# skit-ai/N-Best-ASR-Transformer

Hardware: AMD Instinct MI355X
Metric: utterances/sec fine-tune (bert-base, seq128, n_best=5) (higher is better)
Workload: dtype bf16

## Files before the change

### include/nbest_hip.h

```cpp
#ifndef NBEST_HIP_H
#define NBEST_HIP_H

#include <stddef.h>
#include <stdint.h>

#ifdef __cplusplus
extern "C" {
#endif

#define NBEST_ABI_VERSION 1

enum { NBEST_OK = 0, NBEST_ERR_ARG = -1, NBEST_ERR_SHAPE = -2, NBEST_ERR_DTYPE = -3, NBEST_ERR_ALIGN = -4,
       NBEST_ERR_LAUNCH = -5, NBEST_ERR_WORKSPACE = -6 };
enum { NBEST_F32 = 0, NBEST_BF16 = 1 };

typedef void* nbest_stream_t;

int nbest_version(void);
int nbest_last_error(char* buf, size_t n);

int nbest_embed_ln_fwd(const int64_t* ids, const int64_t* seg, const int64_t* pos, const void* word,
                       const void* type, const void* ptab, const float* gamma, const float* beta, void* out,
                       float* stats, int64_t M, int H, float eps, int dtype, float drop_p, uint64_t seed,
                       uint32_t drop_stream, nbest_stream_t stream);
// ... 61 lines not shown
  int32_t wave_rows, wave_cols;
  int32_t stages;
  int32_t form;
  int32_t reg_epilogue;
  int32_t splits;
  int64_t k_per_split;
  int32_t b_packed;
  int32_t kernel_epilogue;
} nbest_gemm_plan_info;
int nbest_gemm_plan(const nbest_gemm_args* a, nbest_gemm_plan_info* out);

size_t nbest_wgrad_pair_ws_bytes(const nbest_gemm_args* a, const nbest_gemm_args* b);
int nbest_wgrad_pair(const nbest_gemm_args* a, const nbest_gemm_args* b, nbest_stream_t stream);
int nbest_wgrad_group(const nbest_gemm_args* problems, int n, nbest_stream_t stream);
int nbest_wgrad_window(const nbest_gemm_args* problems, const int32_t* tile_first, const int32_t* tile_count, int n, nbest_stream_t stream);

typedef struct nbest_gemm_fp8_args {
  const void* A;
  const void* B;
  void* C;
  const float* bias;
  const void* R;
  void* U;
  void* C8;
  int64_t M, N, K;
  int64_t lda, ldb, ldc, ldr, ldu, ldc8;
  int32_t epilogue;
  float out_scale;
  float drop_p;
  uint32_t drop_stream;
// ... 221 lines not shown
```

### n-best-asr-transformer_amd/csrc/encoder.hip

```cpp
#include <algorithm>
#include <vector>

#include "common.h"

namespace {

static inline size_t al(size_t x) { return (x + 255) & ~(size_t)255; }
static inline size_t take(size_t& o, size_t bytes) { const size_t at = o; o += bytes; return at; }

struct Sizes {
  size_t esz, MH, MF, M3H, MH8, MF8, st, lse;
  int64_t M;
};

static Sizes sizes(const nbest_encoder_desc* d) {
  Sizes z;
  z.esz = d->dtype == NBEST_BF16 ? 2 : 4;
  z.M = (int64_t)d->B * d->S;
  const size_t MHe = (size_t)z.M * d->H, MFe = (size_t)z.M * d->F;
  z.MH = al(MHe * z.esz); z.MF = al(MFe * z.esz); z.M3H = al(3 * MHe * z.esz);
  z.MH8 = al(MHe); z.MF8 = al(MFe);
  z.st = al((size_t)z.M * 2 * sizeof(float));
  z.lse = al((size_t)d->B * d->heads * d->S * sizeof(float));
  return z;
// ... 263 lines not shown
  g.M = M; g.N = N; g.K = K; g.lda = K; g.ldb = K; g.ldc = N;
  return g;
}

static void use_packed(nbest_gemm_args& g, const void* arena, int64_t off) {
  if (!arena || g.dtype != NBEST_BF16 || g.trans_a || g.trans_b) return;
  g.B_packed = (const char*)arena + off * 2;
  g.b_pack_bn = nbest_pack_bn(g.N);
}
static void use_packed(nbest_gemm_fp8_args& g, const void* arena, int64_t off) {
  if (!arena) return;
  g.B_packed = (const uint8_t*)arena + off;
  g.b_pack_bn = nbest_pack_bn_fp8(g.N, g.K);
}

struct GemmPass {
  int dtype; int64_t M; nbest_stream_t stream;
  uint64_t seed;
  Ptrs W; const void* packed; bool b_kn;
  bool fp8; const void *w8, *w8_packed; const float* inv_scale; const uint32_t* amax_prev; uint32_t* amax_new;
  void* colsum_ws; size_t colsum_ws_bytes; int accumulate;
};
struct GemmOp {
  const void* A; const uint8_t* A8; int a_idx;
  int64_t w_off; int mat;
  void* C; int64_t N, K; int epilogue;
  const float* bias;
  const void* R; float drop_p; uint32_t drop_stream;
  void* U; float* colsum;
  uint8_t* C8; int c_idx;
};

static int layer_gemm(const GemmPass& c, const GemmOp& o) {
  if (c.fp8) {
    nbest_gemm_fp8_args g = {};
    g.A = o.A8; g.B = (const uint8_t*)c.w8 + o.w_off; g.C = o.C; g.bias = o.bias; g.R = o.R; g.U = o.U; g.C8 = o.C8;
// ... 7 lines not shown
      g.c8_amax_prev = c.amax_prev + o.c_idx;
      g.c8_amax_new = c.amax_new ? c.amax_new + (int64_t)o.c_idx * NBEST_AMAX_TENSOR_WORDS : nullptr;
    }
    g.colsum_out = o.colsum; g.colsum_accumulate = c.accumulate; g.ws = c.colsum_ws; g.ws_bytes = c.colsum_ws_bytes;
    return nbest_gemm_fp8(&g, c.stream);
  }
  nbest_gemm_args g = gemm_nt(c.dtype, o.A, c.W.W(o.w_off), o.C, c.M, o.N, o.K);
  if (c.b_kn) { g.trans_b = 1; g.ldb = o.N; }
  g.epilogue = o.epilogue; g.bias = o.bias;
  if (o.R) { g.R = o.R; g.ldr = o.N; }
  if (o.epilogue == NBEST_EPI_BIAS_DROP_RES) { g.drop_p = o.drop_p; g.drop_stream = o.drop_stream; g.seed = c.seed; }
  if (o.epilogue == NBEST_EPI_BIAS_GELU || o.epilogue == NBEST_EPI_DGELU) { g.U = o.U; g.ldu = o.N; }
  if (o.epilogue == NBEST_EPI_DGELU) {
    g.colsum_out = o.colsum; g.colsum_accumulate = g.accumulate = c.accumulate; g.ws = c.colsum_ws; g.ws_bytes = c.colsum_ws_bytes;
  }
  use_packed(g, c.packed, o.w_off);
  return nbest_gemm(&g, c.stream);
}

struct LayerBufs {
  void *qkv, *ctx, *r1, *x1, *u, *hact, *r2;
  float *lse, *st1, *st2;
  uint32_t* keep;
  uint8_t *x8, *ctx8, *x18, *h8;
};

static LayerBufs stashed_layer(const nbest_encoder_desc* d, const ActLayout& a, void* act, int l) {
  char* Lb = (char*)act + a.layer0 + (size_t)(l - a.K) * a.layer_stride;
  LayerBufs b = {};
  b.qkv = Lb + a.o_qkv; b.ctx = Lb + a.o_ctx; b.lse = (float*)(Lb + a.o_lse);
// ... 88 lines not shown
  const nbest_layer_offsets& o = d->layers_host[l];
  const Ptrs& P = c.g.W;
  const nbest_stream_t stream = c.g.stream;
  hipStream_t st = (hipStream_t)stream;
  const int H = d->H, F = d->F, dt = d->dtype, t = 4 * l;
  const int64_t B = d->B, SH = (int64_t)d->S * H;
  const uint32_t s0 = d->drop_stream_base + 1 + 4 * l;
  const bool hdrop = d->hidden_drop > 0.f;
  void* tmp = (char*)b.r2 + (size_t)B * H * P.esz;
  const GemmOp wqkv = {xin, nullptr, t + 0, o.wqkv, t + 0, b.qkv, 3 * H, H, NBEST_EPI_BIAS, P.P(o.bqkv)};
  RUN(layer_gemm(c.g, wqkv));
  RUN(nbest_attention_cls_fwd_internal(b.qkv, SH * 3, (const char*)b.qkv + H * P.esz, 3 * H, c.key_mask, b.ctx, H, d->B, d->S, d->heads, 64, dt,
                                       stream, d->attn_drop, d->seed, s0 + 0));
  auto dense_drop_res = [&](const void* A, int64_t w_off, const float* bias, int64_t N, int64_t K, const void* R, int64_t ldr, uint32_t ds,
                            void* out) -> int {
    nbest_gemm_args g = gemm_nt(dt, A, P.W(w_off), hdrop ? tmp : out, B, N, K);
    g.bias = bias;
    if (hdrop) {
      g.epilogue = NBEST_EPI_BIAS;
      RUN(nbest_gemm(&g, stream));
      return nbest_internal_rows_drop_res(tmp, N, R, ldr, out, N, B, (int)N, d->S, dt, d->hidden_drop, d->seed, ds, st);
    }
    g.epilogue = NBEST_EPI_BIAS_DROP_RES; g.R = R; g.ldr = ldr;
    return nbest_gemm(&g, stream);
  };
  RUN(dense_drop_res(b.ctx, o.wo, P.P(o.bo), H, H, xin, SH, s0 + 1, b.r1));
  RUN(nbest_internal_layernorm_fwd8(b.r1, P.P(o.ln1_g), P.P(o.ln1_b), b.x1, nullptr, b.st1, B, H, d->ln_eps, dt, stream, nullptr, nullptr));
  nbest_gemm_args g = gemm_nt(dt, b.x1, P.W(o.w1), b.hact, B, F, H);
  g.epilogue = NBEST_EPI_BIAS_GELU; g.bias = P.P(o.b1); g.U = b.u; g.ldu = F;
  RUN(nbest_gemm(&g, stream));
  RUN(dense_drop_res(b.hact, o.w2, P.P(o.b2), H, F, b.x1, H, s0 + 2, b.r2));
  RUN(nbest_internal_layernorm_fwd8(b.r2, P.P(o.ln2_g), P.P(o.ln2_b), tmp, nullptr, b.st2, B, H, d->ln_eps, dt, stream, nullptr, nullptr));
  return nbest_internal_rows_drop_res(tmp, H, nullptr, 0, xout, SH, B, H, 1, dt, 0.f, 0, 0, st);
}

}

extern "C" size_t nbest_encoder_act_bytes(const nbest_encoder_desc* d) { return d ? act_layout(d, sizes(d)).total : 0; }

extern "C" int nbest_encoder_act_view(const nbest_encoder_desc* d, void* act, int layer, void** qkv, float** lse) {
  RUN(check_desc(d));
  RUN(check_cls_top(d));
  NB_CHECK(act && qkv && lse, NBEST_ERR_ARG, "encoder_act_view: null pointer");
  NB_CHECK(0 <= layer && layer < d->L, NBEST_ERR_ARG, "encoder_act_view: layer %d outside [0, L=%d)", layer, d->L);
  const ActLayout a = act_layout(d, sizes(d));
// ... 203 lines not shown
    void *dR2 = dR, *dR1 = dR, *dRd2 = dRd, *dRd1 = dRd, *dBigL = dBig, *dqkvL = dqkv;
    if (deferred) {
      dRd2 = W + w.gset[gpos][0]; dBigL = W + w.gset[gpos][1]; dRd1 = W + w.gset[gpos][2]; dqkvL = W + w.gset[gpos][3];
      if (!hdrop) { dR2 = dRd2; dR1 = dRd1; }
    }
    const bool cls = cls_layer_of(d, l);
    if (cls) {
      const size_t bh = (size_t)d->B * H * z.esz;
      dR2 = W + w.dR; dR1 = W + w.dB1 + bh; dBigL = dBig;
      dRd2 = hdrop ? (void*)(W + w.dRd) : dR2; dRd1 = hdrop ? (void*)(W + w.dRd + bh) : dR1;
    }
    const WGrad wg[4] = {{dqkvL, X(l), dqkv8, b.x8, o.wqkv, 3 * H, H, t + 3, t + 0},
                         {dRd1, b.ctx, dRd8, b.ctx8, o.wo, H, H, t + 2, t + 1},
                         {dBigL, b.x1, dBig8, b.x18, o.w1, F, H, t + 1, t + 2},
                         {dRd2, b.hact, dRd8, b.h8, o.w2, H, F, t + 0, t + 3}};
    auto cls_wgrad = [&](int j) -> int {
      if (frozen(l, j)) return NBEST_OK;
      nbest_gemm_args g = wgrad_args(dt, wg[j].rows, wg[j].cols, d->B);
      g.A = wg[j].dY; g.B = wg[j].X; g.C = G(wg[j].w_off); g.accumulate = accumulate;
      g.ws = slab; g.ws_bytes = w.slab_bytes;
      return nbest_gemm(&g, stream);
    };
    auto cls_wgrads = [&]() -> int {
      RUN(cls_wgrad(3));
      RUN(cls_wgrad(2));
      return cls_wgrad(1);
    };
    if (!npg) nbest_internal_rowred_batch_begin();
    if (cls) {
      const int64_t Bn = d->B, SH = (int64_t)d->S * H;
      const size_t bh = (size_t)Bn * H * z.esz, half = w.red_bytes / 2;
      void* dAc = W + w.dR + bh;
      GemmPass dgc = dg;
      dgc.M = Bn; dgc.packed = nullptr;
      const Fp8Grad nof8 = {nullptr, nullptr, nullptr};
      RUN(nbest_internal_rows_drop_res(dA, SH, nullptr, 0, dAc, H, Bn, H, 1, dt, 0.f, 0, 0, st));
      RUN(nbest_internal_layernorm_bwd8(dAc, b.r2, b.st2, P.P(o.ln2_g), dR2, nullptr, G(o.ln2_g), G(o.ln2_b), hdrop ? nullptr : G(o.b2), Bn, H, dt,
                                        accumulate, 0.f, 0, 0, red, half, stream, nof8));
      if (hdrop) {
        RUN(nbest_internal_rows_drop_res(dR2, H, nullptr, 0, dRd2, H, Bn, H, d->S, dt, d->hidden_drop, d->seed, s0 + 2, st));
        RUN(nbest_colsum(dRd2, G(o.b2), Bn, H, H, dt, accumulate, (char*)red + half, half, stream));
      }
      GemmOp dw2 = {dRd2, nullptr, t + 0, o.w2, t + 3, dBigL, F, H, NBEST_EPI_DGELU};
      dw2.U = b.u; dw2.colsum = G(o.b1);
      RUN(layer_gemm(dgc, dw2));
      GemmOp dw1 = {dBigL, nullptr, t + 1, o.w1, t + 2, dB1, H, F, NBEST_EPI_RES};
      dw1.R = dR2;
      RUN(layer_gemm(dgc, dw1));
      RUN(nbest_internal_layernorm_bwd8(dB1, b.r1, b.st1, P.P(o.ln1_g), dR1, nullptr, G(o.ln1_g), G(o.ln1_b), hdrop ? nullptr : G(o.bo), Bn, H, dt,
// ... 57 lines not shown
        const WinLaunch& wl = wp.launches[wi];
        nbest_gemm_args tab[kWinEntries];
        int32_t first[kWinEntries], count[kWinEntries];
        for (int i = 0; i < wl.n; ++i) {
          tab[i] = wargs[(size_t)4 * (layer_end - 1 - wl.e[i].layer) + wl.e[i].j];
          first[i] = wl.e[i].first; count[i] = wl.e[i].count;
        }
        pair_begin();
        RUN(nbest_wgrad_window(tab, first, count, wl.n, stream));
        pair_end();
      }
      pair_end();
      if (l == layer_begin)
        for (; pairs_used < nl; ++pairs_used) { stamp(0); stamp(1); }
    } else if (!grouped && cls) {
      stamp(0); RUN(cls_wgrad(3)); stamp(1);
      stamp(0); RUN(cls_wgrad(2)); stamp(1);
      if (!paired) { stamp(0); RUN(cls_wgrad(1)); stamp(1); }
      stamp(0);
      if (paired) RUN(cls_wgrad(1));
      RUN(wgrad_launch(l, wg, 0, -1));
      stamp(1);
    } else if (!grouped) {
      RUN(wgrad(l, wg, 0, paired ? 1 : -1));
    } else if (group_ends && gpos + 1 < gl && d->wgrad_group != NBEST_WGRAD_GROUP_ALWAYS) {
      stamp(0);
      if (cls) RUN(cls_wgrads());
      RUN(wgrad_launch(l, wg, 3, -1));
      RUN(wgrad_launch(l, wg, 2, -1));
      if (!paired) RUN(wgrad_launch(l, wg, 1, -1));
      RUN(wgrad_launch(l, wg, 0, paired ? 1 : -1));
      stamp(1);
    } else {
      for (int j = 0; j < 4; ++j)
        if (!skip(l, j)) pend[n_pend++] = wgrad_args_of(wg + j);
// ... 76 lines not shown
  auto probs = [&](int l) { return cls_attn ? cls_attn + (int64_t)l * B * d->heads * d->S : nullptr; };

  RUN(nbest_embed_ln_fwd(ids, seg, pos, P.W(d->off_word), P.W(d->off_type), P.W(d->off_pos), P.P(d->off_emb_ln_g), P.P(d->off_emb_ln_b),
                         X[0], (float*)(W + w.emb_stats), M, H, d->ln_eps, dt, d->hidden_drop, d->seed, d->drop_stream_base,
                         (hipStream_t)stream));
  for (int l = 0; l + 1 < d->L; ++l) RUN(layer_forward(c, l, X[l & 1], X[(l + 1) & 1], b, nullptr, probs(l)));
  const int l = d->L - 1;
  const nbest_layer_offsets& o = d->layers_host[l];
  const void* xin = X[l & 1];
  void* kv = b.qkv; void* q = b.ctx; void* cctx = b.r1; void* cx1 = b.x1; void* ch = b.hact; void* cr = b.r2;
  nbest_gemm_args g = gemm_nt(dt, xin, P.W(o.wqkv + (int64_t)H * H), kv, M, 2 * H, H);
  g.epilogue = NBEST_EPI_BIAS; g.bias = P.P(o.bqkv + H);
  RUN(nbest_gemm(&g, stream));
  g = gemm_nt(dt, xin, P.W(o.wqkv), q, B, H, H);
  g.lda = SH; g.epilogue = NBEST_EPI_BIAS; g.bias = P.P(o.bqkv);
  RUN(nbest_gemm(&g, stream));
  if (cls_attn) RUN(nbest_internal_attention_cls_probs(q, H, kv, 2 * H, key_mask, probs(l), d->S, d->B, d->S, d->heads, 64, dt, stream));
  RUN(nbest_attention_cls_fwd_internal(q, H, kv, 2 * H, key_mask, cctx, H, d->B, d->S, d->heads, 64, dt, stream, 0.f, 0, 0));
  if (d->head_gate) RUN(nbest_head_gate_fwd(cctx, H, cctx, H, d->head_gate + (int64_t)l * d->heads, B, d->heads, 64, dt, stream));
  g = gemm_nt(dt, cctx, P.W(o.wo), cr, B, H, H);
  g.epilogue = NBEST_EPI_BIAS_DROP_RES; g.bias = P.P(o.bo); g.R = xin; g.ldr = SH;
  RUN(nbest_gemm(&g, stream));
  RUN(nbest_internal_layernorm_fwd8(cr, P.P(o.ln1_g), P.P(o.ln1_b), cx1, nullptr, b.st1, B, H, d->ln_eps, dt, stream, nullptr, nullptr));
  g = gemm_nt(dt, cx1, P.W(o.w1), ch, B, F, H);
  g.epilogue = NBEST_EPI_BIAS_GELU; g.bias = P.P(o.b1); g.ldu = F;
  RUN(nbest_gemm(&g, stream));
  g = gemm_nt(dt, ch, P.W(o.w2), cr, B, H, F);
  g.epilogue = NBEST_EPI_BIAS_DROP_RES; g.bias = P.P(o.b2); g.R = cx1; g.ldr = H;
  RUN(nbest_gemm(&g, stream));
  RUN(nbest_internal_layernorm_fwd8(cr, P.P(o.ln2_g), P.P(o.ln2_b), cls_out, nullptr, b.st2, B, H, d->ln_eps, dt, stream, nullptr, nullptr));
  return NBEST_OK;
}

extern "C" int nbest_encoder_infer(const nbest_encoder_desc* d, const void* wts, const float* prm, const int64_t* ids, const int64_t* seg,
                                   const int64_t* pos, const uint8_t* key_mask, void* ws, size_t ws_bytes, void* cls_out,
                                   nbest_stream_t stream) {
  return nbest_encoder_infer_attn(d, wts, prm, ids, seg, pos, key_mask, ws, ws_bytes, cls_out, nullptr, stream);
}
```

### n-best-asr-transformer_amd/hipabi.py

```python
import collections
import ctypes as C
import os

import torch

_HERE = os.path.dirname(os.path.abspath(__file__))
LIB_PATH = os.environ.get("NBEST_LIB") or os.path.join(_HERE, "csrc", "libnbest_hip.so")

F32, BF16 = 0, 1
ADAM_L2, ADAMW = 0, 1
EPI_NONE, EPI_BIAS, EPI_BIAS_GELU, EPI_BIAS_DROP_RES, EPI_DGELU, EPI_RES, EPI_F32_SPLITK = range(7)

EXPORTS = [
    "nbest_version", "nbest_last_error", "nbest_embed_ln_fwd", "nbest_embed_ln_bwd", "nbest_embed_bwd_ws_bytes", "nbest_rows_gather", "nbest_rows_zero", "nbest_rows_add",
    "nbest_gemm_ws_bytes", "nbest_gemm", "nbest_gemm_plan", "nbest_wgrad_pair_ws_bytes", "nbest_wgrad_pair", "nbest_wgrad_group", "nbest_wgrad_window", "nbest_pack_bn", "nbest_pack_weights", "nbest_pack_bn_fp8", "nbest_pack_weights_fp8", "nbest_attention_fwd", "nbest_attention_bwd", "nbest_attention_bwd_ws_bytes", "nbest_attention_keep_bytes", "nbest_attention_fwd_keep", "nbest_attention_bwd_keep", "nbest_layernorm_fwd",
    "nbest_layernorm_bwd", "nbest_rowred_ws_bytes", "nbest_colsum", "nbest_heads_ws_bytes", "nbest_stc_heads", "nbest_stc_heads_kd", "nbest_stc_heads_kd_t", "nbest_stc_heads_logits", "nbest_stc_heads_rdrop",
    "nbest_stc_heads_vjp", "nbest_cls_mse", "nbest_cls_grad_scatter", "nbest_stc_decode", "nbest_stream_stamp", "nbest_fp8_amax_fold", "nbest_bertadam_chunk", "nbest_bertadam_step", "nbest_bertadam_norms", "nbest_bertadam_update",
    "nbest_adam_clip_coef", "nbest_adam_update", "nbest_adam_step", "nbest_ema_update", "nbest_ema_exchange",
    "nbest_cast_f32_to_bf16", "nbest_transpose_weights", "nbest_encoder_act_bytes", "nbest_encoder_ws_bytes", "nbest_encoder_wgrad_launches_per_layer", "nbest_encoder_wgrad_plan", "nbest_encoder_forward",
    "nbest_encoder_backward", "nbest_gemm_fp8", "nbest_gemm_fp8_ws_bytes", "nbest_wgrad_fp8", "nbest_wgrad_fp8_ws_bytes", "nbest_wgrad_fp8_pair", "nbest_wgrad_fp8_pair_ws_bytes", "nbest_cast_bf16_to_fp8", "nbest_quantize_weights_fp8",
    "nbest_attention_cls_fwd", "nbest_encoder_infer_ws_bytes", "nbest_encoder_infer",
    "nbest_attention_probs", "nbest_attention_cls_probs", "nbest_encoder_act_view", "nbest_encoder_infer_attn",
    "nbest_embed_ln_fwd_interp", "nbest_embed_attrib",
    "nbest_head_gate_fwd", "nbest_head_gate_bwd",
]


class GemmArgs(C.Structure):
    _fields_ = [("A", C.c_void_p), ("B", C.c_void_p), ("C", C.c_void_p), ("bias", C.c_void_p), ("R", C.c_void_p),
                ("U", C.c_void_p), ("ws", C.c_void_p), ("ws_bytes", C.c_size_t),
# ... 77 lines not shown
                     "nbest_encoder_act_bytes", "nbest_encoder_ws_bytes", "nbest_encoder_infer_ws_bytes"):
            getattr(L, name).restype = C.c_size_t
        L.nbest_embed_bwd_ws_bytes.argtypes = [C.c_int64, C.c_int64]
        L.nbest_rows_gather.argtypes = [C.c_void_p, C.c_void_p, C.c_int64, C.c_int64, C.c_void_p, C.c_void_p, C.c_int, C.c_void_p]
        L.nbest_rows_zero.argtypes = [C.c_void_p, C.c_void_p, C.c_int64, C.c_int, C.c_void_p]
        L.nbest_rows_add.argtypes = [C.c_void_p, C.c_void_p, C.c_void_p, C.c_int64, C.c_int, C.c_void_p]
        L.nbest_rowred_ws_bytes.argtypes = [C.c_int64, C.c_int64]
        L.nbest_heads_ws_bytes.argtypes = [C.c_int, C.c_int, C.c_int]
        L.nbest_gemm_ws_bytes.argtypes = [C.POINTER(GemmArgs)]
        L.nbest_gemm.argtypes = [C.POINTER(GemmArgs), C.c_void_p]
        L.nbest_gemm_plan.argtypes = [C.POINTER(GemmArgs), C.POINTER(GemmPlanInfo)]
        L.nbest_wgrad_pair_ws_bytes.argtypes = [C.POINTER(GemmArgs), C.POINTER(GemmArgs)]
        L.nbest_wgrad_pair.argtypes = [C.POINTER(GemmArgs), C.POINTER(GemmArgs), C.c_void_p]
        L.nbest_wgrad_group.argtypes = [C.POINTER(GemmArgs), C.c_int32, C.c_void_p]
        L.nbest_wgrad_window.argtypes = [C.POINTER(GemmArgs), C.POINTER(C.c_int32), C.POINTER(C.c_int32), C.c_int32, C.c_void_p]
        L.nbest_encoder_act_bytes.argtypes = [C.POINTER(EncoderDesc)]
        L.nbest_encoder_ws_bytes.argtypes = [C.POINTER(EncoderDesc)]
        L.nbest_encoder_wgrad_launches_per_layer.argtypes = [C.POINTER(EncoderDesc)]
        L.nbest_encoder_wgrad_plan.argtypes = [C.POINTER(EncoderDesc), C.c_int32, C.c_int32, C.POINTER(C.c_int32), C.c_int32]
        vp, i64, i32, f32, u64, u32, sz = C.c_void_p, C.c_int64, C.c_int, C.c_float, C.c_uint64, C.c_uint32, C.c_size_t
        L.nbest_embed_ln_fwd.argtypes = [vp] * 10 + [i64, i32, f32, i32, f32, u64, u32, vp]
        L.nbest_embed_ln_bwd.argtypes = [vp] * 15 + [i32, i32, i32, i32, i32, i64, i64, i32, i32, f32, u64, u32, vp, sz, vp]
        L.nbest_embed_ln_fwd_interp.argtypes = [vp] * 12 + [i32, i32, i32, f32, i32, f32, u64, u32, vp]
        L.nbest_embed_attrib.argtypes = [vp] * 11 + [i32, i32, i32, i32, f32, i32, vp]
        L.nbest_head_gate_fwd.argtypes = [vp, i64, vp, i64, vp, i64, i32, i32, i32, vp]
        L.nbest_head_gate_bwd.argtypes = [vp, vp, vp, vp, i32, i32, i32, i32, i32, vp]
        L.nbest_attention_fwd.argtypes = [vp] * 4 + [i32] * 5 + [f32, u64, u32, vp]
        L.nbest_attention_bwd.argtypes = [vp] * 7 + [i32, vp, sz] + [i32] * 5 + [f32, u64, u32, vp]
        L.nbest_attention_bwd_ws_bytes.argtypes = [i32, i32, i32]
        L.nbest_attention_keep_bytes.argtypes = [i32, i32, i32]
# ... 155 lines not shown
    nb = lib().nbest_gemm_ws_bytes(C.byref(g))
    ws = _ws(nb, dev)
    g.ws, g.ws_bytes = ws.data_ptr(), ws.numel()
    return g, out, U, ws


def gemm(A, B, M, N, K, trans_a=False, trans_b=False, epilogue=EPI_NONE, bias=None, R=None, U=None, out=None,
         accumulate=False, drop_p=0.0, seed=0, drop_stream=0, colsum_out=None, defer_reduce=False, B_packed=None, b_pack_bn=0,
         want_u=True):
    g, out, U, ws = _gemm_args(A, B, M, N, K, trans_a, trans_b, epilogue, bias, R, U, out, accumulate, drop_p, seed, drop_stream,
                               colsum_out, defer_reduce, B_packed, b_pack_bn, want_u)
    check(lib().nbest_gemm(C.byref(g), stream_ptr()), "gemm")
    return (out, U) if epilogue == EPI_BIAS_GELU and want_u else out


FORM_NN, FORM_NT, FORM_TT, FORM_TN = range(4)
EPI_BIAS_GELU_NO_U = 0x102


def gemm_plan_args(g):
    info = GemmPlanInfo()
    check(lib().nbest_gemm_plan(C.byref(g), C.byref(info)), "gemm_plan")
    return {name: int(getattr(info, name)) for name, _ in GemmPlanInfo._fields_}


def gemm_plan(A, B, M, N, K, trans_a=False, trans_b=False, epilogue=EPI_NONE, bias=None, R=None, U=None, out=None,
              accumulate=False, drop_p=0.0, seed=0, drop_stream=0, colsum_out=None, defer_reduce=False, B_packed=None, b_pack_bn=0,
              want_u=True):
    g, out, U, ws = _gemm_args(A, B, M, N, K, trans_a, trans_b, epilogue, bias, R, U, out, accumulate, drop_p, seed, drop_stream,
                               colsum_out, defer_reduce, B_packed, b_pack_bn, want_u)
# ... 506 lines not shown
```

Measured before the change: 13370.

## Add split-K small-M GEMM kernel for CLS-only layers and group CLS wgrads

```diff
diff --git a/include/nbest_hip.h b/include/nbest_hip.h
--- a/include/nbest_hip.h
+++ b/include/nbest_hip.h
@@ -99,6 +99,10 @@
 int nbest_wgrad_pair(const nbest_gemm_args* a, const nbest_gemm_args* b, nbest_stream_t stream);
 int nbest_wgrad_group(const nbest_gemm_args* problems, int n, nbest_stream_t stream);
 int nbest_wgrad_window(const nbest_gemm_args* problems, const int32_t* tile_first, const int32_t* tile_count, int n, nbest_stream_t stream);
+
+size_t nbest_gemm_rows_ws_bytes(const nbest_gemm_args* a);
+int nbest_gemm_rows(const nbest_gemm_args* a, nbest_stream_t stream);
+int nbest_gemm_rows_mult(const nbest_gemm_args* a, int64_t drop_row_mult, nbest_stream_t stream);
 
 typedef struct nbest_gemm_fp8_args {
   const void* A;
diff --git a/n-best-asr-transformer_amd/csrc/encoder.hip b/n-best-asr-transformer_amd/csrc/encoder.hip
--- a/n-best-asr-transformer_amd/csrc/encoder.hip
+++ b/n-best-asr-transformer_amd/csrc/encoder.hip
@@ -301,12 +301,19 @@
   g.b_pack_bn = nbest_pack_bn_fp8(g.N, g.K);
 }
 
+static bool rows_refused(int rc) { return rc == NBEST_ERR_DTYPE || rc == NBEST_ERR_SHAPE || rc == NBEST_ERR_ALIGN || rc == NBEST_ERR_WORKSPACE; }
+static int gemm_few_rows(const nbest_gemm_args& g, nbest_stream_t stream) {
+  const int rc = nbest_gemm_rows(&g, stream);
+  return rows_refused(rc) ? nbest_gemm(&g, stream) : rc;
+}
+
 struct GemmPass {
   int dtype; int64_t M; nbest_stream_t stream;
   uint64_t seed;
   Ptrs W; const void* packed; bool b_kn;
   bool fp8; const void *w8, *w8_packed; const float* inv_scale; const uint32_t* amax_prev; uint32_t* amax_new;
   void* colsum_ws; size_t colsum_ws_bytes; int accumulate;
+  bool few_rows;
 };
 struct GemmOp {
   const void* A; const uint8_t* A8; int a_idx;
@@ -344,6 +351,7 @@
   if (o.epilogue == NBEST_EPI_DGELU) {
     g.colsum_out = o.colsum; g.colsum_accumulate = g.accumulate = c.accumulate; g.ws = c.colsum_ws; g.ws_bytes = c.colsum_ws_bytes;
   }
+  if (c.few_rows) return gemm_few_rows(g, c.stream);
   use_packed(g, c.packed, o.w_off);
   return nbest_gemm(&g, c.stream);
 }
@@ -462,6 +470,11 @@
                                        stream, d->attn_drop, d->seed, s0 + 0));
   auto dense_drop_res = [&](const void* A, int64_t w_off, const float* bias, int64_t N, int64_t K, const void* R, int64_t ldr, uint32_t ds,
                             void* out) -> int {
+    nbest_gemm_args r = gemm_nt(dt, A, P.W(w_off), out, B, N, K);
+    r.bias = bias; r.epilogue = NBEST_EPI_BIAS_DROP_RES; r.R = R; r.ldr = ldr;
+    r.drop_p = d->hidden_drop; r.seed = d->seed; r.drop_stream = ds;
+    const int rc = nbest_gemm_rows_mult(&r, d->S, stream);
+    if (!rows_refused(rc)) return rc;
     nbest_gemm_args g = gemm_nt(dt, A, P.W(w_off), hdrop ? tmp : out, B, N, K);
     g.bias = bias;
     if (hdrop) {
@@ -476,7 +489,7 @@
   RUN(nbest_internal_layernorm_fwd8(b.r1, P.P(o.ln1_g), P.P(o.ln1_b), b.x1, nullptr, b.st1, B, H, d->ln_eps, dt, stream, nullptr, nullptr));
   nbest_gemm_args g = gemm_nt(dt, b.x1, P.W(o.w1), b.hact, B, F, H);
   g.epilogue = NBEST_EPI_BIAS_GELU; g.bias = P.P(o.b1); g.U = b.u; g.ldu = F;
-  RUN(nbest_gemm(&g, stream));
+  RUN(gemm_few_rows(g, stream));
   RUN(dense_drop_res(b.hact, o.w2, P.P(o.b2), H, F, b.x1, H, s0 + 2, b.r2));
   RUN(nbest_internal_layernorm_fwd8(b.r2, P.P(o.ln2_g), P.P(o.ln2_b), tmp, nullptr, b.st2, B, H, d->ln_eps, dt, stream, nullptr, nullptr));
   return nbest_internal_rows_drop_res(tmp, H, nullptr, 0, xout, SH, B, H, 1, dt, 0.f, 0, 0, st);
@@ -710,17 +723,27 @@
                          {dRd1, b.ctx, dRd8, b.ctx8, o.wo, H, H, t + 2, t + 1},
                          {dBigL, b.x1, dBig8, b.x18, o.w1, F, H, t + 1, t + 2},
                          {dRd2, b.hact, dRd8, b.h8, o.w2, H, F, t + 0, t + 3}};
-    auto cls_wgrad = [&](int j) -> int {
-      if (frozen(l, j)) return NBEST_OK;
+    auto cls_wgrad_args = [&](int j) {
       nbest_gemm_args g = wgrad_args(dt, wg[j].rows, wg[j].cols, d->B);
       g.A = wg[j].dY; g.B = wg[j].X; g.C = G(wg[j].w_off); g.accumulate = accumulate;
-      g.ws = slab; g.ws_bytes = w.slab_bytes;
-      return nbest_gemm(&g, stream);
+      return g;
     };
     auto cls_wgrads = [&]() -> int {
-      RUN(cls_wgrad(3));
-      RUN(cls_wgrad(2));
-      return cls_wgrad(1);
+      nbest_gemm_args tab[3];
+      int n = 0;
+      bool whole = dt == NBEST_BF16;
+      for (int j = 3; j >= 1; --j) {
+        if (frozen(l, j)) continue;
+        tab[n] = cls_wgrad_args(j);
+        whole = whole && tab[n].M % 256 == 0 && tab[n].N % 256 == 0;
+        ++n;
+      }
+      if (n && whole) return nbest_wgrad_group(tab, n, stream);
+      for (int i = 0; i < n; ++i) {
+        tab[i].ws = slab; tab[i].ws_bytes = w.slab_bytes;
+        RUN(nbest_gemm(&tab[i], stream));
+      }
+      return NBEST_OK;
     };
     if (!npg) nbest_internal_rowred_batch_begin();
     if (cls) {
@@ -728,7 +751,7 @@
       const size_t bh = (size_t)Bn * H * z.esz, half = w.red_bytes / 2;
       void* dAc = W + w.dR + bh;
       GemmPass dgc = dg;
-      dgc.M = Bn; dgc.packed = nullptr;
+      dgc.M = Bn; dgc.packed = nullptr; dgc.few_rows = true;
       const Fp8Grad nof8 = {nullptr, nullptr, nullptr};
       RUN(nbest_internal_rows_drop_res(dA, SH, nullptr, 0, dAc, H, Bn, H, 1, dt, 0.f, 0, 0, st));
       RUN(nbest_internal_layernorm_bwd8(dAc, b.r2, b.st2, P.P(o.ln2_g), dR2, nullptr, G(o.ln2_g), G(o.ln2_b), hdrop ? nullptr : G(o.b2), Bn, H, dt,
@@ -816,11 +839,10 @@
       if (l == layer_begin)
         for (; pairs_used < nl; ++pairs_used) { stamp(0); stamp(1); }
     } else if (!grouped && cls) {
-      stamp(0); RUN(cls_wgrad(3)); stamp(1);
-      stamp(0); RUN(cls_wgrad(2)); stamp(1);
-      if (!paired) { stamp(0); RUN(cls_wgrad(1)); stamp(1); }
+      stamp(0); RUN(cls_wgrads()); stamp(1);
+      stamp(0); stamp(1);
+      if (!paired) { stamp(0); stamp(1); }
       stamp(0);
-      if (paired) RUN(cls_wgrad(1));
       RUN(wgrad_launch(l, wg, 0, -1));
       stamp(1);
     } else if (!grouped) {
@@ -927,20 +949,20 @@
   RUN(nbest_gemm(&g, stream));
   g = gemm_nt(dt, xin, P.W(o.wqkv), q, B, H, H);
   g.lda = SH; g.epilogue = NBEST_EPI_BIAS; g.bias = P.P(o.bqkv);
-  RUN(nbest_gemm(&g, stream));
+  RUN(gemm_few_rows(g, stream));
   if (cls_attn) RUN(nbest_internal_attention_cls_probs(q, H, kv, 2 * H, key_mask, probs(l), d->S, d->B, d->S, d->heads, 64, dt, stream));
   RUN(nbest_attention_cls_fwd_internal(q, H, kv, 2 * H, key_mask, cctx, H, d->B, d->S, d->heads, 64, dt, stream, 0.f, 0, 0));
   if (d->head_gate) RUN(nbest_head_gate_fwd(cctx, H, cctx, H, d->head_gate + (int64_t)l * d->heads, B, d->heads, 64, dt, stream));
   g = gemm_nt(dt, cctx, P.W(o.wo), cr, B, H, H);
   g.epilogue = NBEST_EPI_BIAS_DROP_RES; g.bias = P.P(o.bo); g.R = xin; g.ldr = SH;
-  RUN(nbest_gemm(&g, stream));
+  RUN(gemm_few_rows(g, stream));
   RUN(nbest_internal_layernorm_fwd8(cr, P.P(o.ln1_g), P.P(o.ln1_b), cx1, nullptr, b.st1, B, H, d->ln_eps, dt, stream, nullptr, nullptr));
   g = gemm_nt(dt, cx1, P.W(o.w1), ch, B, F, H);
   g.epilogue = NBEST_EPI_BIAS_GELU; g.bias = P.P(o.b1); g.ldu = F;
-  RUN(nbest_gemm(&g, stream));
+  RUN(gemm_few_rows(g, stream));
   g = gemm_nt(dt, ch, P.W(o.w2), cr, B, H, F);
   g.epilogue = NBEST_EPI_BIAS_DROP_RES; g.bias = P.P(o.b2); g.R = cx1; g.ldr = H;
-  RUN(nbest_gemm(&g, stream));
+  RUN(gemm_few_rows(g, stream));
   RUN(nbest_internal_layernorm_fwd8(cr, P.P(o.ln2_g), P.P(o.ln2_b), cls_out, nullptr, b.st2, B, H, d->ln_eps, dt, stream, nullptr, nullptr));
   return NBEST_OK;
 }
diff --git a/n-best-asr-transformer_amd/csrc/gemm_rows.hip b/n-best-asr-transformer_amd/csrc/gemm_rows.hip
--- /dev/null
+++ b/n-best-asr-transformer_amd/csrc/gemm_rows.hip
@@ -0,0 +1,276 @@
+#include "common.h"
+
+namespace {
+
+constexpr int kMaxRows = 512;
+constexpr int BM = 32, BN = 32, BK = 64;
+constexpr int depth_of(int kw) { return kw == 8 ? 4 : 3; }
+constexpr uint32_t kOob = 0x80000000u;
+
+struct RowsP {
+  const bf16* A; const bf16* B; bf16* C; const float* bias; const bf16* R; uint8_t* U; float* colpart;
+  uint32_t a_bytes, b_bytes, c_bytes, r_bytes, u_bytes;
+  uint32_t lda2, ldb2, ldc2, ldr2, ldu;
+  int M, N, K, tiles_m;
+  uint32_t drop_row;
+  DropCfg drop;
+};
+
+struct Frag { u32x4 a[4], b[4]; };
+constexpr int kTile = BM * BK * 2;
+
+template <int KW, int EPI>
+__global__ __launch_bounds__(KW * 64) void gemm_rows_kernel(RowsP p) {
+  __shared__ __attribute__((aligned(16))) char stage[KW][2][kTile];
+  __shared__ float colred[2][BN];
+  const int tid = threadIdx.x, lane = tid & 63, wave = tid >> 6;
+  const int lr = lane & 15, g = lane >> 4;
+  const int id = xcd_remap(blockIdx.x, gridDim.x);
+  const int strip = id / p.tiles_m, tm = id - strip * p.tiles_m;
+  const int m0 = tm * BM, n0 = strip * BN;
+
+  constexpr uint32_t kFlags = 0x00020000;
+  const __amdgpu_buffer_rsrc_t rsA = __builtin_amdgcn_make_buffer_rsrc((void*)p.A, 0, p.a_bytes, kFlags);
+  const __amdgpu_buffer_rsrc_t rsB = __builtin_amdgcn_make_buffer_rsrc((void*)p.B, 0, p.b_bytes, kFlags);
+  const __amdgpu_buffer_rsrc_t rsC = __builtin_amdgcn_make_buffer_rsrc((void*)p.C, 0, p.c_bytes, kFlags);
+
+  constexpr bool kHasBias = (EPI == NBEST_EPI_BIAS || EPI == NBEST_EPI_BIAS_GELU || EPI == kEpiBiasGeluNoU || EPI == NBEST_EPI_BIAS_DROP_RES);
+  constexpr bool kHasR = (EPI == NBEST_EPI_BIAS_DROP_RES || EPI == NBEST_EPI_RES);
+  const bool ep_thread = wave < 4;
+  const int ei = (wave >> 1) & 1, ej = wave & 1;
+  const uint32_t em = (uint32_t)(m0 + ei * 16 + lr), en = (uint32_t)(n0 + ej * 16 + g * 4);
+  f32x4 pb = {0, 0, 0, 0};
+  u32x2 pr = {0, 0};
+  uint32_t pu = 0;
+  if (ep_thread) {
+    if (kHasBias) pb = *(const f32x4*)(p.bias + en);
+    if (kHasR) {
+      const __amdgpu_buffer_rsrc_t rsR = __builtin_amdgcn_make_buffer_rsrc((void*)p.R, 0, p.r_bytes, kFlags);
+      pr = __builtin_amdgcn_raw_buffer_load_b64(rsR, em * p.ldr2 + en * 2, 0, 0);
+    }
+    if (EPI == NBEST_EPI_DGELU) {
+      const __amdgpu_buffer_rsrc_t rsU = __builtin_amdgcn_make_buffer_rsrc((void*)p.U, 0, p.u_bytes, kFlags);
+      pu = __builtin_amdgcn_raw_buffer_load_b32(rsU, em * p.ldu + en, 0, 0);
+    }
+  }
+
+  const int steps = p.K / BK, per = (steps + KW - 1) / KW;
+  const int sbeg = wave * per;
+  const int nst = (sbeg + per <= steps) ? per : (steps > sbeg ? steps - sbeg : 0);
+  uint32_t offA[4], offB[4], wr[4], rd[2][2];
+#pragma unroll
+  for (int i = 0; i < 4; ++i) {
+    const int row = i * 8 + (lane >> 3), slot = lane & 7;
+    offA[i] = (uint32_t)(m0 + row) * p.lda2 + (uint32_t)(sbeg * BK + slot * 8) * 2;
+    offB[i] = (uint32_t)(n0 + row) * p.ldb2 + (uint32_t)(sbeg * BK + slot * 8) * 2;
+    wr[i] = (uint32_t)(row * 128 + ((slot ^ ((row >> 1) & 7)) << 4));
+  }
+#pragma unroll
+  for (int t = 0; t < 2; ++t)
+#pragma unroll
+    for (int ks = 0; ks < 2; ++ks) {
+      const int row = t * 16 + lr, kc = g + 4 * ks;
+      rd[t][ks] = (uint32_t)(row * 128 + ((kc ^ ((row >> 1) & 7)) << 4));
+    }
+  char* const myA = stage[wave][0];
+  char* const myB = stage[wave][1];
+  auto load = [&](Frag& f, int s) {
+    const bool ok = s < nst;
+    const uint32_t ko = (uint32_t)s * (BK * 2);
+#pragma unroll
+    for (int i = 0; i < 4; ++i) {
+      f.a[i] = __builtin_amdgcn_raw_buffer_load_b128(rsA, ok ? offA[i] + ko : kOob, 0, 0);
+      f.b[i] = __builtin_amdgcn_raw_buffer_load_b128(rsB, ok ? offB[i] + ko : kOob, 0, 0);
+    }
+  };
+
+  f32x4 acc[2][2];
+#pragma unroll
+  for (int i = 0; i < 2; ++i)
+#pragma unroll
+    for (int j = 0; j < 2; ++j) acc[i][j] = f32x4{0, 0, 0, 0};
+
+  constexpr int kDepth = depth_of(KW);
+  Frag f[kDepth];
+#pragma unroll
+  for (int d = 0; d < kDepth; ++d) load(f[d], d);
+  for (int s = 0; s < nst; s += kDepth) {
+#pragma unroll
+    for (int d = 0; d < kDepth; ++d) {
+#pragma unroll
+      for (int i = 0; i < 4; ++i) {
+        *(u32x4*)(myA + wr[i]) = f[d].a[i];
+        *(u32x4*)(myB + wr[i]) = f[d].b[i];
+      }
+      load(f[d], s + d + kDepth);
+      __builtin_amdgcn_wave_barrier();
+      bf16x8 af[2][2], bfr[2][2];
+#pragma unroll
+      for (int t = 0; t < 2; ++t)
+#pragma unroll
+        for (int ks = 0; ks < 2; ++ks) {
+          af[t][ks] = *(const bf16x8*)(myA + rd[t][ks]);
+          bfr[t][ks] = *(const bf16x8*)(myB + rd[t][ks]);
+        }
+      __builtin_amdgcn_wave_barrier();
+#pragma unroll
+      for (int ks = 0; ks < 2; ++ks)
+#pragma unroll
+        for (int i = 0; i < 2; ++i)
+#pragma unroll
+          for (int j = 0; j < 2; ++j)
+            acc[i][j] = __builtin_amdgcn_mfma_f32_16x16x32_bf16(bfr[j][ks], af[i][ks], acc[i][j], 0, 0, 0);
+    }
+  }
+
+#pragma unroll
+  for (int i = 0; i < 2; ++i)
+#pragma unroll
+    for (int j = 0; j < 2; ++j) ((f32x4*)stage[wave][0])[(i * 2 + j) * 64 + lane] = acc[i][j];
+  __syncthreads();
+  float x[4] = {0, 0, 0, 0};
+  if (ep_thread) {
+    f32x4 t = ((const f32x4*)stage[0][0])[wave * 64 + lane];
+#pragma unroll
+    for (int w = 1; w < KW; ++w) t += ((const f32x4*)stage[w][0])[wave * 64 + lane];
+    float v[4] = {t[0], t[1], t[2], t[3]};
+    if (kHasBias) {
+#pragma unroll
+      for (int e = 0; e < 4; ++e) v[e] += pb[e];
+    }
+    if (EPI == kEpiBiasGeluNoU) {
+#pragma unroll
+      for (int e = 0; e < 4; e += 2) {
+        f32x2 h2, g2;
+        gelu_pair_fast(f32x2{v[e], v[e + 1]}, h2, g2);
+        v[e] = h2[0]; v[e + 1] = h2[1];
+      }
+    }
+    if (EPI == NBEST_EPI_BIAS_GELU) {
+      float gp[4];
+#pragma unroll
+      for (int e = 0; e < 4; e += 2) {
+        f32x2 h2, g2;
+        gelu_pair_fast(f32x2{v[e], v[e + 1]}, h2, g2);
+        gp[e] = g2[0]; gp[e + 1] = g2[1]; v[e] = h2[0]; v[e + 1] = h2[1];
+      }
+      const __amdgpu_buffer_rsrc_t rsU = __builtin_amdgcn_make_buffer_rsrc((void*)p.U, 0, p.u_bytes, kFlags);
+      __builtin_amdgcn_raw_buffer_store_b32(gd_pack4(gp), rsU, em * p.ldu + en, 0, 2 );
+    }
+    if (EPI == NBEST_EPI_BIAS_DROP_RES) {
+      if (p.drop.thr16) {
+        const uint32_t k = nb_keep4(p.drop, em * p.drop_row + en);
+#pragma unroll
+        for (int e = 0; e < 4; ++e) v[e] = (k >> e & 1) ? v[e] * p.drop.scale : 0.f;
+      }
+    }
+    if (kHasR) {
+      const bf16x4 r = __builtin_bit_cast(bf16x4, pr);
+#pragma unroll
+      for (int e = 0; e < 4; ++e) v[e] += (float)r[e];
+    }
+    if (EPI == NBEST_EPI_DGELU) {
+      float gd[4];
+      gd_unpack4(pu, gd);
+#pragma unroll
+      for (int e = 0; e < 4; ++e) v[e] *= gd[e];
+    }
+    bf16x4 o;
+#pragma unroll
+    for (int e = 0; e < 4; ++e) { o[e] = (bf16)v[e]; x[e] = (em < (uint32_t)p.M) ? v[e] : 0.f; }
+    const u32x2 ow = __builtin_bit_cast(u32x2, o);
+    nb_bstore8(rsC, em * p.ldc2 + en * 2, ow[0], ow[1]);
+  }
+  if (p.colpart) {
+#pragma unroll
+    for (int e = 0; e < 4; ++e) {
+      float s = x[e];
+      s += __shfl_xor(s, 1, 64); s += __shfl_xor(s, 2, 64); s += __shfl_xor(s, 4, 64); s += __shfl_xor(s, 8, 64);
+      x[e] = s;
+    }
+    if (ep_thread && lr == 0) *(f32x4*)&colred[ei][ej * 16 + g * 4] = f32x4{x[0], x[1], x[2], x[3]};
+    __syncthreads();
+    if (tid < BN) p.colpart[(int64_t)tm * p.N + n0 + tid] = colred[0][tid] + colred[1][tid];
+  }
+}
+
+template <int KW>
+static int launch_epi(const RowsP& p, int epi, int grid, hipStream_t st) {
+#define L(E)                                                \
+  case E:                                                   \
+    gemm_rows_kernel<KW, E><<<grid, KW * 64, 0, st>>>(p);   \
+    break;
+  switch (epi) {
+    L(NBEST_EPI_NONE) L(NBEST_EPI_BIAS) L(NBEST_EPI_BIAS_GELU) L(NBEST_EPI_BIAS_DROP_RES) L(NBEST_EPI_DGELU) L(NBEST_EPI_RES)
+    L(kEpiBiasGeluNoU)
+    default:
+      nbest_set_error("gemm_rows: bad epilogue %d", epi);
+      return NBEST_ERR_ARG;
+  }
+#undef L
+  NB_LAUNCH_CHECK();
+  return NBEST_OK;
+}
+
+static int check_rows(const nbest_gemm_args* a, int64_t drop_row_mult) {
+  NB_CHECK(a && a->A && a->B && a->C, NBEST_ERR_ARG, "gemm_rows: null pointer");
+  NB_CHECK(a->dtype == NBEST_BF16, NBEST_ERR_DTYPE, "gemm_rows: bf16 only (dtype %d)", a->dtype);
+  NB_CHECK(a->M > 0 && a->M <= kMaxRows, NBEST_ERR_SHAPE, "gemm_rows: M=%lld outside 1 .. %d", (long long)a->M, kMaxRows);
+  NB_CHECK(a->N > 0 && a->N % 128 == 0, NBEST_ERR_SHAPE, "gemm_rows: N=%lld must be a multiple of 128", (long long)a->N);
+  NB_CHECK(a->K > 0 && a->K % BK == 0, NBEST_ERR_SHAPE, "gemm_rows: K=%lld must be a multiple of %d", (long long)a->K, BK);
+  NB_CHECK(!a->trans_a && !a->trans_b, NBEST_ERR_SHAPE, "gemm_rows: both operands must be k-contiguous (trans_a = trans_b = 0)");
+  const int epi = a->epilogue;
+  NB_CHECK(epi >= NBEST_EPI_NONE && epi <= NBEST_EPI_RES, NBEST_ERR_ARG, "gemm_rows: epilogue %d is not built", epi);
+  NB_CHECK(a->lda >= a->K && a->ldb >= a->K && a->ldc >= a->N, NBEST_ERR_ARG, "gemm_rows: a leading dimension is shorter than its row");
+  NB_CHECK(a->lda % 8 == 0 && a->ldb % 8 == 0 && a->ldc % 8 == 0, NBEST_ERR_ALIGN, "gemm_rows: leading dimensions must be multiples of 8");
+  NB_CHECK(((uintptr_t)a->A & 15) == 0 && ((uintptr_t)a->B & 15) == 0 && ((uintptr_t)a->C & 15) == 0, NBEST_ERR_ALIGN,
+           "gemm_rows: pointers must be 16-byte aligned");
+  const bool bias = epi == NBEST_EPI_BIAS || epi == NBEST_EPI_BIAS_GELU || epi == NBEST_EPI_BIAS_DROP_RES;
+  const bool res = epi == NBEST_EPI_BIAS_DROP_RES || epi == NBEST_EPI_RES;
+  const bool u = (epi == NBEST_EPI_BIAS_GELU && a->U) || epi == NBEST_EPI_DGELU;
+  NB_CHECK(!bias || (a->bias && ((uintptr_t)a->bias & 15) == 0), NBEST_ERR_ARG, "gemm_rows: epilogue %d needs a 16-byte aligned bias", epi);
+  NB_CHECK(!res || (a->R && a->ldr >= a->N && a->ldr % 8 == 0 && ((uintptr_t)a->R & 15) == 0), NBEST_ERR_ARG, "gemm_rows: epilogue %d needs R", epi);
+  NB_CHECK(!u || (a->U && a->ldu >= a->N && a->ldu % 8 == 0 && ((uintptr_t)a->U & 15) == 0), NBEST_ERR_ARG, "gemm_rows: epilogue %d needs U", epi);
+  const int64_t rows = round_up(a->M, BM), lim = (int64_t)1 << 31;
+  NB_CHECK(rows * a->lda * 2 < lim && a->N * a->ldb * 2 < lim && rows * a->ldc * 2 < lim && (!res || rows * a->ldr * 2 < lim) &&
+               (!u || rows * a->ldu < lim),
+           NBEST_ERR_SHAPE, "gemm_rows: an operand spans 2 GiB or more");
+  if (epi == NBEST_EPI_BIAS_DROP_RES && make_drop(a->drop_p, a->seed, a->drop_stream).thr16)
+    NB_CHECK(drop_row_mult >= 1 && a->M * drop_row_mult * a->N < ((int64_t)1 << 32), NBEST_ERR_SHAPE, "gemm_rows: dropout counter overflow");
+  if (a->colsum_out)
+    NB_CHECK(a->ws && ((uintptr_t)a->ws & 15) == 0 && a->ws_bytes >= nbest_gemm_rows_ws_bytes(a), NBEST_ERR_WORKSPACE,
+             "gemm_rows: column-sum workspace too small");
+  return NBEST_OK;
+}
+
+}
+
+extern "C" size_t nbest_gemm_rows_ws_bytes(const nbest_gemm_args* a) {
+  if (!a || !a->colsum_out || a->M <= 0 || a->N <= 0) return 0;
+  return (size_t)((a->M + BM - 1) / BM) * a->N * sizeof(float);
+}
+
+extern "C" int nbest_gemm_rows_mult(const nbest_gemm_args* a, int64_t drop_row_mult, nbest_stream_t stream) {
+  if (int rc = check_rows(a, drop_row_mult)) return rc;
+  hipStream_t st = (hipStream_t)stream;
+  RowsP p;
+  p.A = (const bf16*)a->A; p.B = (const bf16*)a->B; p.C = (bf16*)a->C; p.bias = a->bias; p.R = (const bf16*)a->R; p.U = (uint8_t*)a->U;
+  p.colpart = a->colsum_out ? (float*)a->ws : nullptr;
+  p.a_bytes = (uint32_t)(((a->M - 1) * a->lda + a->K) * 2);
+  p.b_bytes = (uint32_t)(((a->N - 1) * a->ldb + a->K) * 2);
+  p.c_bytes = (uint32_t)(((a->M - 1) * a->ldc + a->N) * 2);
+  p.r_bytes = a->R ? (uint32_t)(((a->M - 1) * a->ldr + a->N) * 2) : 0;
+  p.u_bytes = a->U ? (uint32_t)((a->M - 1) * a->ldu + a->N) : 0;
+  p.lda2 = (uint32_t)(a->lda * 2); p.ldb2 = (uint32_t)(a->ldb * 2); p.ldc2 = (uint32_t)(a->ldc * 2); p.ldr2 = (uint32_t)(a->ldr * 2);
+  p.ldu = (uint32_t)a->ldu;
+  p.M = (int)a->M; p.N = (int)a->N; p.K = (int)a->K; p.tiles_m = (int)((a->M + BM - 1) / BM);
+  p.drop = make_drop(a->drop_p, a->seed, a->drop_stream);
+  p.drop_row = (uint32_t)(drop_row_mult * a->N);
+  const int grid = p.tiles_m * (int)(a->N / BN);
+  const int kepi = nb_kernel_epilogue(a->epilogue, a->U);
+  if (int rc = (a->K >= 1536) ? launch_epi<8>(p, kepi, grid, st) : launch_epi<4>(p, kepi, grid, st)) return rc;
+  if (p.colpart) return nbest_internal_partial_rows_sum(p.colpart, p.tiles_m, (int)a->N, a->colsum_out, a->colsum_accumulate, st);
+  return NBEST_OK;
+}
+
+extern "C" int nbest_gemm_rows(const nbest_gemm_args* a, nbest_stream_t stream) { return nbest_gemm_rows_mult(a, 1, stream); }
diff --git a/n-best-asr-transformer_amd/hipabi.py b/n-best-asr-transformer_amd/hipabi.py
--- a/n-best-asr-transformer_amd/hipabi.py
+++ b/n-best-asr-transformer_amd/hipabi.py
@@ -13,7 +13,7 @@
 
 EXPORTS = [
     "nbest_version", "nbest_last_error", "nbest_embed_ln_fwd", "nbest_embed_ln_bwd", "nbest_embed_bwd_ws_bytes", "nbest_rows_gather", "nbest_rows_zero", "nbest_rows_add",
-    "nbest_gemm_ws_bytes", "nbest_gemm", "nbest_gemm_plan", "nbest_wgrad_pair_ws_bytes", "nbest_wgrad_pair", "nbest_wgrad_group", "nbest_wgrad_window", "nbest_pack_bn", "nbest_pack_weights", "nbest_pack_bn_fp8", "nbest_pack_weights_fp8", "nbest_attention_fwd", "nbest_attention_bwd", "nbest_attention_bwd_ws_bytes", "nbest_attention_keep_bytes", "nbest_attention_fwd_keep", "nbest_attention_bwd_keep", "nbest_layernorm_fwd",
+    "nbest_gemm_ws_bytes", "nbest_gemm", "nbest_gemm_plan", "nbest_wgrad_pair_ws_bytes", "nbest_wgrad_pair", "nbest_wgrad_group", "nbest_wgrad_window", "nbest_gemm_rows_ws_bytes", "nbest_gemm_rows", "nbest_gemm_rows_mult", "nbest_pack_bn", "nbest_pack_weights", "nbest_pack_bn_fp8", "nbest_pack_weights_fp8", "nbest_attention_fwd", "nbest_attention_bwd", "nbest_attention_bwd_ws_bytes", "nbest_attention_keep_bytes", "nbest_attention_fwd_keep", "nbest_attention_bwd_keep", "nbest_layernorm_fwd",
     "nbest_layernorm_bwd", "nbest_rowred_ws_bytes", "nbest_colsum", "nbest_heads_ws_bytes", "nbest_stc_heads", "nbest_stc_heads_kd", "nbest_stc_heads_kd_t", "nbest_stc_heads_logits", "nbest_stc_heads_rdrop",
     "nbest_stc_heads_vjp", "nbest_cls_mse", "nbest_cls_grad_scatter", "nbest_stc_decode", "nbest_stream_stamp", "nbest_fp8_amax_fold", "nbest_bertadam_chunk", "nbest_bertadam_step", "nbest_bertadam_norms", "nbest_bertadam_update",
     "nbest_adam_clip_coef", "nbest_adam_update", "nbest_adam_step", "nbest_ema_update", "nbest_ema_exchange",
@@ -121,6 +121,10 @@
         L.nbest_wgrad_pair.argtypes = [C.POINTER(GemmArgs), C.POINTER(GemmArgs), C.c_void_p]
         L.nbest_wgrad_group.argtypes = [C.POINTER(GemmArgs), C.c_int32, C.c_void_p]
         L.nbest_wgrad_window.argtypes = [C.POINTER(GemmArgs), C.POINTER(C.c_int32), C.POINTER(C.c_int32), C.c_int32, C.c_void_p]
+        L.nbest_gemm_rows_ws_bytes.restype = C.c_size_t
+        L.nbest_gemm_rows_ws_bytes.argtypes = [C.POINTER(GemmArgs)]
+        L.nbest_gemm_rows.argtypes = [C.POINTER(GemmArgs), C.c_void_p]
+        L.nbest_gemm_rows_mult.argtypes = [C.POINTER(GemmArgs), C.c_int64, C.c_void_p]
         L.nbest_encoder_act_bytes.argtypes = [C.POINTER(EncoderDesc)]
         L.nbest_encoder_ws_bytes.argtypes = [C.POINTER(EncoderDesc)]
         L.nbest_encoder_wgrad_launches_per_layer.argtypes = [C.POINTER(EncoderDesc)]
@@ -306,6 +310,60 @@
     return (out, U) if epilogue == EPI_BIAS_GELU and want_u else out
 
 
+GEMM_ROWS_MAX_M = 512
+
+
+def gemm_rows_args(M, N, K, epilogue=EPI_NONE, dtype=BF16, lda=None, ldb=None, ldc=None, ldr=None, ldu=None, with_u=True, colsum=False):
+    g = GemmArgs()
+    fake = 1 << 20
+    g.A, g.B, g.C = fake, fake, fake
+    g.M, g.N, g.K = M, N, K
+    g.lda, g.ldb, g.ldc = (lda or K), (ldb or K), (ldc or N)
+    g.epilogue, g.dtype = epilogue, dtype
+    if epilogue in (EPI_BIAS, EPI_BIAS_GELU, EPI_BIAS_DROP_RES):
+        g.bias = fake
+    if epilogue in (EPI_BIAS_DROP_RES, EPI_RES):
+        g.R, g.ldr = fake, (ldr or N)
+    if epilogue == EPI_DGELU or (epilogue == EPI_BIAS_GELU and with_u):
+        g.U, g.ldu = fake, (ldu or N)
+    if colsum:
+        g.colsum_out = fake
+        g.ws, g.ws_bytes = fake, max(int(lib().nbest_gemm_rows_ws_bytes(C.byref(g))), 16)
+    return g
+
+
+def gemm_rows_rc(g, drop_row_mult=1):
+    stream = stream_ptr() if torch.cuda.is_available() else C.c_void_p(0)
+    return int(lib().nbest_gemm_rows_mult(C.byref(g), int(drop_row_mult), stream))
+
+
+def gemm_rows(A, B, M, N, K, epilogue=EPI_NONE, bias=None, R=None, U=None, out=None, drop_p=0.0, seed=0, drop_stream=0,
+              drop_row_mult=1, colsum_out=None, colsum_accumulate=False, want_u=True):
+    dev = A.device
+    if out is None:
+        out = torch.empty(M, N, dtype=A.dtype, device=dev)
+    if epilogue == EPI_BIAS_GELU and U is None and want_u:
+        U = torch.empty(M, N, dtype=torch.uint8, device=dev)
+    g = GemmArgs()
+    g.A, g.B, g.C = A.data_ptr(), B.data_ptr(), out.data_ptr()
+    g.bias = bias.data_ptr() if bias is not None else None
+    g.R = R.data_ptr() if R is not None else None
+    g.U = U.data_ptr() if U is not None else None
+    g.M, g.N, g.K = M, N, K
+    g.lda, g.ldb, g.ldc = A.stride(0), B.stride(0), out.stride(0)
+    g.ldr = R.stride(0) if R is not None else 0
+    g.ldu = U.stride(0) if U is not None else 0
+    g.epilogue, g.dtype = epilogue, dtype_code(A.dtype)
+    g.drop_p, g.drop_stream, g.seed = drop_p, drop_stream, seed
+    ws = None
+    if colsum_out is not None:
+        g.colsum_out, g.colsum_accumulate = colsum_out.data_ptr(), int(colsum_accumulate)
+        ws = _ws(lib().nbest_gemm_rows_ws_bytes(C.byref(g)), dev)
+        g.ws, g.ws_bytes = ws.data_ptr(), ws.numel()
+    check(lib().nbest_gemm_rows_mult(C.byref(g), int(drop_row_mult), stream_ptr()), "gemm_rows")
+    return (out, U) if epilogue == EPI_BIAS_GELU and want_u else out
+
+
 FORM_NN, FORM_NT, FORM_TT, FORM_TN = range(4)
 EPI_BIAS_GELU_NO_U = 0x102
 
```

Result: no change. 13470, median of 6 (+0.7%).
